# salesforce/warp-drive

Measured on AMD Instinct MI355X. Metric: env steps/sec, TagContinuous 5 taggers x 100 runners, higher is better.
Workload: dtype f32; 1 GPU; BASELINE configs[2]: TagContinuous 5 taggers x 100 runners, partial obs K=10 (F=71), num_envs=2000 per GPU; tick = sample_actions (2 heads) + step + reset of finished replicas (one fused launch); num_envs_per_gpu=2000, num_agents=105, launch_mode=plan, kernels_per_tick=1, ticks_per_launch=1, parallelism=env-replica sharding x1

## Files before the change

### warp_drive_amd/csrc/kernels/tc_fast.h

```cpp
#pragma once
#include "wd_common.h"
#include "tc_fetch.h"
#include "tc_sample.h"
#include "tc_move.h"
#include "tc_tags.h"
#include "tc_reset.h"
#include "tc_knn.h"
#include "tc_rows.h"

namespace {

template <int KMAX, bool FUSED, bool EXACTK, int IDB, bool SAMPLE = FUSED, bool LOOP = false, int SN = 0, int SA = 0,
          int ST = 0>
__device__ __forceinline__ int tc_fast_impl(const TcArgs &a, const TcFuse &fz, unsigned char *smem, int n_acc,
                                            int n_turn, int tick = 0, int n_taggers_in = 0, TcCarry *cy = nullptr,
                                            const TcLoopConsts *lc = nullptr) {
  WD_TC_PROBE_TICK(LOOP, tick);
  const int N = a.N, K = EXACTK ? KMAX : a.K;
  const int F = 7 * K + 1;
  int tid_ = threadIdx.x;
  if constexpr (LOOP) asm volatile("" : "+v"(tid_));
  const int tid = tid_, T_ = WD_TC_BLOCKDIM;
  const int epb = max(1, T_ / N);
  const int n_waves = (T_ + 63) >> 6, wave = __builtin_amdgcn_readfirstlane(tid >> 6), lane = tid & 63;
  const size_t slab_acc_bytes = tc_align16((size_t)4 * epb * N * n_acc);
  const bool compact = (epb == 1);
  const size_t slab_turn_bytes = tc_align16((size_t)4 * epb * N * n_turn);
  const bool one_slab = tc_one_slab(N);
  const TcFastLds l = tc_carve_fast(smem, epb, N, K, n_waves,
                                    !SAMPLE ? 0 : one_slab ? max(slab_acc_bytes, slab_turn_bytes) : slab_acc_bytes + slab_turn_bytes,
                                    compact);
  const TcTables &tb = l.tb;
  float *const slab_acc = (float *)smem, *const slab_turn = (float *)(smem + (one_slab ? 0 : slab_acc_bytes));
  float *const stage = l.stage + (size_t)wave * l.stage_dwords;
  const int el = tid / N, ag = tid - el * N;
  const float invK = 1.0f / (float)K, invN = 1.0f / (float)N;
  const int NP = ((N + 3) & ~3) + 8;

  int group = blockIdx.x;
#ifndef WD_TC_BLOCK_ORDER_PLAIN
  if constexpr (IDB == 7) {
    const int bx = blockIdx.x & 7, bq = gridDim.x >> 3, br = gridDim.x & 7;
    group = bx * bq + min(bx, br) + (int)(blockIdx.x >> 3);
  }
#endif
  const int env0 = a.env_begin + group * epb;
  __builtin_amdgcn_s_setprio(3);
  WD_TC_PROBE_RT(16); WD_TC_PROBE(0); WD_TC_PROBE_HW(21);
  TcIn in;
  bool reloaded = false;
  if constexpr (LOOP) {
    in = cy->in;
    reloaded = cy->reload != 0;
    if (reloaded) {
      tc_load_state(in, a, fz, env0, epb, N, n_acc, n_turn, tid, tick == 0);
      cy->in.type = in.type; cy->in.skill = in.skill; cy->in.step_reward = in.step_reward;
    }
  } else {
    tc_issue_loads<FUSED, SAMPLE>(in, a, fz, env0, epb, N, n_acc, n_turn, tid, slab_acc, slab_turn, true);
  }
  const bool tab_in_lds = (n_acc <= WD_TC_TAB) && (n_turn <= WD_TC_TAB);
  int n_taggers_ = n_taggers_in;
  if constexpr (LOOP) {
    if (tick == 0) n_taggers_ = tc_build_tables(tb, a, N, n_acc, n_turn, tab_in_lds, in);
  } else {
    n_taggers_ = tc_build_tables(tb, a, N, n_acc, n_turn, tab_in_lds, in);
  }
  const int n_taggers = n_taggers_;
  if (env0 >= a.E) return n_taggers;
  if constexpr (!LOOP) WD_TC_PROBE(1);

  const int env = env0 + el;
  const bool active = (el < epb) && (env < a.E);
  const int gi = env * N + ag;
  const int li = tid;
  const int agents_here = min(epb, a.E - env0) * N;
  if constexpr (LOOP) {
    if (active && ag == 0) a.done[env] = 0;
    static_assert(!LOOP || (SN > 0 && SA > 0 && ST == WD_TC_BLOCKDIM), "the multi-tick entry is built for one shape");
    tc_fetch_slabs_straight<SN, SA, ST>(slab_acc, slab_turn, fz.probs_acc, fz.probs_turn, env0, wave, lane);
    WD_TC_PROBE(1);
  }
  int2 sampled = in.sampled;
  const unsigned long long live_mask = __ballot(active && in.sg != 0);
  if constexpr (!LOOP) {
    if (compact && lane == 0) tb.live_cnt[wave] = __popcll(live_mask);
  }
  if constexpr ((IDB != 7) && (KMAX <= 12)) {
    if (compact && tid < 64) tb.cell_cnt[tid] = 0;
  }
  if constexpr (LOOP) {
    static_assert(!LOOP || IDB == 7, "tc_sample_heads_carried samples from two slabs: replicas of at most 128 agents");
    sampled = tc_sample_heads_carried<SA>(fz, in.epoch, cy->k0, cy->k1, active, gi, li, slab_acc, slab_turn, n_acc, n_turn);
    if (compact && lane == 0) tb.live_cnt[wave] = __popcll(live_mask);
  } else if (FUSED) {
    if (active && ag == 0) a.done[env] = 0;
    if (SAMPLE) sampled = tc_sample_heads(a, fz, in, active, gi, li, slab_acc, slab_turn, n_acc, n_turn, env0, epb);
  }
  WD_TC_PROBE(2);
  __syncthreads();
  WD_TC_PROBE(3);
  int my_c = ag, n_live = N;
  if (compact) {
    int before = 0;
    n_live = 0;
    for (int w2 = 0; w2 < n_waves; ++w2) {
      const int c = tb.live_cnt[w2];
      before += (w2 < wave) ? c : 0;
      n_live += c;
    }
    my_c = before + __popcll(live_mask & ((1ull << lane) - 1ull));
  }
  constexpr bool PRE = (IDB != 7) && (KMAX <= 12);
  constexpr bool TIE_TABLE = (IDB != 7);
  bool pre_on = false;
  int cells_C = 0;
  float cell_len = 0.0f, cell_inv = 0.0f;
  int my_cell = 0, my_cell_slot = 0;
  uint4 hint_a = make_uint4(~0u, ~0u, ~0u, ~0u), hint_b = hint_a;
  if constexpr (PRE) {
    pre_on = compact && (a.knn_prev != nullptr) && (n_live >= WD_TC_PRE_MIN_LIVE) && (l.stage_dwords >= WD_TC_LIST_DWORDS);
    if (pre_on && active && in.sg != 0) {
      const uint4 *const h = (const uint4 *)(a.knn_prev + (size_t)(env * N + ag) * 8);
      hint_a = h[0];
      hint_b = h[1];
    }
    if (pre_on) {
      cells_C = tc_cell_grid(n_live, K);
      cell_len = a.grid_length / (float)max(cells_C, 1);
      cell_inv = (float)cells_C / a.grid_length;
    }
  }

  float edge_pen = 0.0f, my_x = 0.0f, my_y = 0.0f;
  const int sg = in.sg;
  const bool is_runner = active && (in.type == 0) && (sg != 0);
  if (active) {
    const TcMoved m = tc_move<LOOP>(a, tb, in, sampled, gi, tab_in_lds, LOOP ? cy : nullptr, LOOP ? lc : nullptr);
    edge_pen = m.edge_pen; my_x = m.x; my_y = m.y;
    if constexpr (LOOP) {
      cy->in.x = m.x; cy->in.y = m.y;
      cy->in.cleared = (sg == 0) ? 1 : 0;
    }
    l.xy[el * NP + ag] = make_float2(sg ? m.x : (PRE && pre_on ? __builtin_nanf("") : WD_BIG), m.y);
    if (compact) {
      if (sg) {
        bool by_cell = false;
        if constexpr (PRE) {
          if (cells_C != 0) {
            const int2 c = tc_cell_xy(m.x, m.y, cell_inv, cells_C);
            my_cell = tc_cell_place(c, cells_C);
            my_cell_slot = atomicAdd(&tb.cell_cnt[my_cell], 1);
            by_cell = true;
          }
        }
        if (!by_cell) {
          l.xyc[my_c] = make_float2(m.x, m.y);
          l.cid[1 + my_c] = (short)ag;
          if (PRE && pre_on) {
            uint4 *const slot = (uint4 *)(l.stage + (size_t)(my_c >> 6) * l.stage_dwords) + 2 * (my_c & 63);
            slot[0] = hint_a;
            slot[1] = hint_b;
          }
        }
      }
      if (ag == 0) {
        l.cid[0] = -1;
        if (PRE && pre_on) {
          l.xyc[n_live] = make_float2(WD_BIG, WD_BIG);
          l.xy[N] = make_float2(__builtin_nanf(""), 0.0f);
        }
      }
    }
    tc_feat_store(l.feat, li, m.ft);
    l.sig[li] = (sg ? 1 : 0) | (in.cleared ? 2 : 0);
    if ((in.cleared != 0) != (sg == 0)) a.obs_rows_cleared[gi] = sg ? 0 : 1;
    l.tagcnt[li] = 0;
    if (ag == 0) {
      const int t = in.tstep + 1;
      a.timestep[env] = t;
      tb.tstep[el] = t;
      if constexpr (LOOP) tb.tfrac[el] = (float)tc_div_const((double)t, (double)a.T, lc->r_T);
      else tb.tfrac[el] = (float)((double)t / (double)a.T);
      if constexpr (LOOP) {
        cy->in.tstep = t;
        if (reloaded) tb.nrun[el] = in.nrun;
      } else {
        tb.nrun[el] = in.nrun;
      }
    }
  }
  WD_TC_PROBE(4);
  __syncthreads();
  WD_TC_PROBE(5);
  int cell_incl = 0;
  if constexpr (PRE) {
    if (cells_C != 0) {
      const int cnt = tb.cell_cnt[lane];
      cell_incl = cnt;
#pragma unroll
      for (int d = 1; d < 64; d <<= 1) {
        const int up = __shfl_up(cell_incl, d, 64);
        cell_incl += (lane >= d) ? up : 0;
      }
      my_c = __builtin_amdgcn_ds_bpermute(my_cell << 2, cell_incl - cnt) + my_cell_slot;
      if (active && sg != 0) {
        l.xyc[my_c] = make_float2(my_x, my_y);
        l.cid[1 + my_c] = (short)ag;
        uint4 *const slot = (uint4 *)(l.stage + (size_t)(my_c >> 6) * l.stage_dwords) + 2 * (my_c & 63);
        slot[0] = hint_a;
        slot[1] = hint_b;
      }
    }
  }

  bool tagged = false;
  if constexpr (LOOP) {
    if (is_runner)
      tagged = tc_find_tag<true>(a, tb, l.xy + el * NP, l.tagcnt + el * N, &tb.nrun[el], n_taggers, my_x, my_y, lc->Bc);
  } else {
    if (is_runner)
      tagged = tc_find_tag(a, tb, l.xy + el * NP, l.tagcnt + el * N, &tb.nrun[el], n_taggers, my_x, my_y);
  }
  if constexpr (PRE) {
    if (cells_C != 0) __syncthreads();
  }

  WD_TC_PROBE(6);
  int nid[KMAX + 1], rank[KMAX + 1];
#pragma unroll
  for (int k = 0; k <= KMAX; ++k) { nid[k] = -1; rank[k] = k; }
  bool in_order = true;
  __builtin_amdgcn_s_setprio(2);
  const bool searcher = compact ? (tid < n_live) : (active && sg != 0);
  const float2 *const sxy = compact ? l.xyc : l.xy + el * NP;
  const int n_cand = compact ? n_live : N;
  int row_agent = ag;
  constexpr int L = KMAX + ((EXACTK && IDB == 7) ? 2 : 3);
  const bool split = compact && (n_waves == 2) && (n_live <= 64) && (n_live >= 16) &&
                     (l.stage_dwords >= 64 * L);
  const int j_half = split ? (((n_live + 7) >> 3) << 2) : n_cand;
  const bool helper = split && (wave == 1);
  unsigned S[L];
  bool prefiltered = false;
  unsigned extra = 0xffffffffu;
  if constexpr (PRE) {
    if (pre_on) {
      unsigned Tb = 0u;
      float sx = 0.0f, sy = 0.0f;
      int2 scell = make_int2(0, 0);
      if (searcher) {
        const uint4 *const slot = (const uint4 *)stage + 2 * lane;
        const uint4 pa = slot[0], pb = slot[1];
        sx = sxy[ag].x; sy = sxy[ag].y;
        Tb = tc_knn_bound16<KMAX>(l.xy, N, sx, sy, pa, pb, K);
        if (cells_C != 0) {
          scell = tc_cell_xy(sx, sy, cell_inv, cells_C);
          Tb = min(Tb, tc_cell_cover2(sx, sy, scell, cell_len, cells_C));
        }
      }
      WD_TC_PROBE(7);
      if (__ballot(searcher) != 0ull && __ballot(searcher && Tb == 0x7f800000u) == 0ull) {
        const float Tf = searcher ? __uint_as_float(Tb) : -1.0f;
#pragma unroll
        for (int k = 0; k < L; ++k) S[k] = 0xffffffffu;
        const int C = cells_C;
        int r = 0, r_end = -1, run0 = 0, run1 = n_cand, x_lo = 0, y_lo = 0, x_hi = 0, y_hi = 0;
        if (C != 0) {
          const int last = min(63, __builtin_amdgcn_readfirstlane(n_live) - 1 - 64 * wave);
          x_lo = __builtin_amdgcn_readfirstlane(scell.x); y_lo = __builtin_amdgcn_readfirstlane(scell.y);
          x_hi = __builtin_amdgcn_readlane(scell.x, last); y_hi = __builtin_amdgcn_readlane(scell.y, last);
          r = max(0, y_lo - 1);
          r_end = min(C - 1, y_hi + 1);
          run1 = 0;
        }
        const TcPreList pl = tc_pre_list(stage, lane);
        int j = 0, j_end = 0;
        int listed = 0, words = 0;
        int probe_trips = 0;
        bool finished = false;
        while (!finished) {
          while (words < WD_TC_LIST_CAP) {
            if (j >= j_end) {
              bool flush = false;
              int p0 = 0, p1 = 0;
              while (!flush && r <= r_end) {
                int lo = C, hi = -1;
                for (int yy = max(y_lo, r - 1); yy <= min(y_hi, r + 1); ++yy) {
                  const bool fwd = (yy & 1) == 0;
                  const int from = (yy == y_lo) ? x_lo : (fwd ? 0 : C - 1), to = (yy == y_hi) ? x_hi : (fwd ? C - 1 : 0);
                  lo = min(lo, min(from, to));
                  hi = max(hi, max(from, to));
                }
                lo = max(0, lo - 1);
                hi = min(C - 1, hi + 1);
                const int first_cell = r * C + ((r & 1) ? C - 1 - hi : lo), last_cell = r * C + ((r & 1) ? C - 1 - lo : hi);
                ++r;
                if (hi < lo) continue;
                const int b = first_cell == 0 ? 0 : __builtin_amdgcn_readlane(cell_incl, max(first_cell, 1) - 1);
                const int e = __builtin_amdgcn_readlane(cell_incl, last_cell);
                const int j0 = max(run1, b & ~3), j1 = min(n_cand, (e + 3) & ~3);
                if (j1 <= j0) continue;
                if (run1 > run0 && j0 != run1) { p0 = run0; p1 = run1; flush = true; run0 = j0; run1 = j1; }
                else if (run1 > run0) run1 = j1;
                else { run0 = j0; run1 = j1; }
              }
              if (!flush) {
                if (run1 <= run0) { finished = true; break; }
                p0 = run0; p1 = run1; run0 = run1;
              }
              j = p0;
              j_end = p1;
            }
            const int j_stop = min(j_end, j + 32 * (WD_TC_LIST_CAP - words));
            tc_pre_pass1(sxy, sx, sy, j, j_stop, Tf, pl, listed);
            words += (j_stop - j + 31) >> 5;
            j = j_stop;
          }
          if (words != 0) tc_pre_pass2<L, IDB>(sxy, sx, sy, pl, listed, S, extra, probe_trips);
          listed = 0;
          words = 0;
        }
        WD_TC_PROBE_VAL(18, probe_trips);
        unsigned sK = S[KMAX];
#pragma unroll
        for (int k = 1; k < KMAX; ++k) sK = (k == K) ? S[k] : sK;
        const bool held = (sK >> IDB) + 2u <= (Tb >> IDB);
        prefiltered = __ballot(searcher && !held) == 0ull;
        WD_TC_PROBE_VAL(19, prefiltered ? 1 : 2);
        if (!prefiltered) extra = 0xffffffffu;
      }
      WD_TC_PROBE(8);
    }
  }
  if (!prefiltered && (searcher || (helper && lane < n_live))) {
    const int me = helper ? lane : ag;
    tc_chain_range<L, IDB>(sxy, sxy[me].x, sxy[me].y, helper ? j_half : 0, helper ? n_cand : j_half, S);
  }
  WD_TC_PROBE(9);
  if (split) {
    if (helper && lane < n_live) {
#pragma unroll
      for (int k = 0; k < L; ++k) ((unsigned *)stage)[64 * k + lane] = S[k];
      __builtin_amdgcn_s_setprio(0);
    }
    __syncthreads();
    if (searcher) {
      const unsigned *const theirs = (const unsigned *)(l.stage + (size_t)l.stage_dwords);
      unsigned P[L];
#pragma unroll
      for (int k = 0; k < L; ++k) P[k] = theirs[64 * k + lane];
      tc_merge_sorted<L>(S, P);
    }
  }
  bool exact = true;
  unsigned zone_hi = 0u;
  if (searcher) {
    unsigned o[L - 1];
    __builtin_amdgcn_s_setprio(1);
    exact = tc_resolve_keys<KMAX, IDB, L, TIE_TABLE>(sxy, ag, K, S, o, nid, rank, in_order, l.cid);
    WD_TC_PROBE(10);
    {
      unsigned oKth = o[KMAX - 1];
#pragma unroll
      for (int k = 0; k < KMAX - 1; ++k) oKth = (k == K - 1) ? o[k] : oKth;
      zone_hi = (oKth >> IDB) + 1u;
    }
    if constexpr (PRE) {
      if (pre_on) {
        unsigned w[8];
#pragma unroll
        for (int q = 0; q < 8; ++q) {
          unsigned pair = 0u;
#pragma unroll
          for (int h = 0; h < 2; ++h) {
            const int k = 2 * q + h;
            const unsigned key = (k < L - 1) ? o[k < L - 1 ? k : 0] : (k == L - 1) ? extra : 0xffffffffu;
            const unsigned id = (key >= 0x7f800000u) ? 0xffffu : (unsigned)(unsigned short)l.cid[1 + (key & ((1u << IDB) - 1u))];
            pair |= id << (16 * h);
          }
          w[q] = pair;
        }
        uint4 *const h = (uint4 *)(a.knn_prev + (size_t)(env * N + l.cid[1 + ag]) * 8);
        h[0] = make_uint4(w[0], w[1], w[2], w[3]);
        h[1] = make_uint4(w[4], w[5], w[6], w[7]);
      }
    }
    if (!exact && !(EXACTK && IDB == 7) && (IDB == 7 || n_cand <= 128)) {
      WD_TC_PROBE_VAL(20, 1);
      int nid2[KMAX], rank2[KMAX];
#pragma unroll
      for (int k = 0; k < KMAX; ++k) { nid2[k] = -1; rank2[k] = k; }
      tc_knn_registers<KMAX>(sxy, ag, n_cand, K, nid2, rank2);
#pragma unroll
      for (int k = 0; k < KMAX; ++k) { nid[k] = nid2[k]; rank[k] = rank2[k]; }
      nid[KMAX] = -1;
      rank[KMAX] = KMAX;
      in_order = false;
      exact = true;
    }
  }
  if constexpr (IDB != 7 || EXACTK) {
    unsigned long long need = __ballot(searcher && !exact);
    if (need != 0ull) {
      WD_TC_PROBE_VAL(20, 1);
      unsigned long long unresolved = 0ull;
      const float mx = searcher ? sxy[ag].x : 0.0f, my = searcher ? sxy[ag].y : 0.0f;
      while (need != 0ull) {
        const int fl = __ffsll((long long)need) - 1;
        need &= need - 1ull;
        const float sx = __builtin_bit_cast(float, __builtin_amdgcn_readlane(__builtin_bit_cast(int, mx), fl));
        const float sy = __builtin_bit_cast(float, __builtin_amdgcn_readlane(__builtin_bit_cast(int, my), fl));
        const unsigned zh = (unsigned)__builtin_amdgcn_readlane((int)zone_hi, fl);
        const int self = __builtin_amdgcn_readlane(ag, fl);
        const float2 *const zxy = compact ? sxy : l.xy + __builtin_amdgcn_readlane(el, fl) * NP;
        const int cnt = tc_zone_resolve<TIE_TABLE>(zxy, n_cand, sx, sy, self, zh, IDB, K, (unsigned char *)stage, lane, l.cid);
        if (cnt > 64) {
          unresolved |= 1ull << fl;
        } else {
          const unsigned short *const out = (const unsigned short *)((const unsigned char *)stage + 128 + 512);
#pragma unroll
          for (int k = 0; k < KMAX; ++k) {
            const int v = (k < K) ? (int)out[k] : -1;
            if (lane == fl) { nid[k] = v; rank[k] = k; }
          }
          if (lane == fl) { nid[KMAX] = -1; rank[KMAX] = KMAX; in_order = false; }
        }
        asm volatile("" ::: "memory");
        __builtin_amdgcn_wave_barrier();
      }
      if ((unresolved >> lane) & 1ull) {
        int nid2[KMAX];
#pragma unroll
        for (int k = 0; k < KMAX; ++k) nid2[k] = -1;
        tc_knn_scan<KMAX, TIE_TABLE>(sxy, ag, n_cand, K, nid2, l.cid);
#pragma unroll
        for (int k = 0; k < KMAX; ++k) { nid[k] = nid2[k]; rank[k] = k; }
        nid[KMAX] = -1;
        rank[KMAX] = KMAX;
        in_order = false;
      }
    }
  }
  if (searcher && compact) {
    row_agent = l.cid[1 + ag];
#pragma unroll
    for (int k = 0; k <= KMAX; ++k) nid[k] = l.cid[1 + nid[k]];
  }
  __builtin_amdgcn_s_setprio(0);
  WD_TC_PROBE(11);

  if constexpr (LOOP) {
    static_assert(!LOOP || (EXACTK && KMAX == 10 && IDB == 7), "the id rows of the multi-tick entry are built for K = 10");
    const bool any_out_of_order = __ballot(!in_order) != 0ull;
    if (searcher) {
      unsigned *const idrow = (unsigned *)(l.ids + row_agent * KMAX);
#pragma unroll
      for (int k = 0; k < KMAX; k += 2) idrow[k >> 1] = ((unsigned)nid[k] & 0xffffu) | ((unsigned)nid[k + 1] << 16);
      if (any_out_of_order && !in_order) {
        unsigned short *const hrow = l.ids + row_agent * KMAX;
#pragma unroll
        for (int k = 0; k <= KMAX; ++k)
          if (rank[k] < KMAX) hrow[rank[k]] = (unsigned short)(nid[k] < 0 ? 0xffff : nid[k]);
#pragma unroll
        for (int k = 0; k < KMAX; ++k) nid[k] = (int)((const short *)hrow)[k];
      }
      tc_store_id_row<false>(a.nearest_ids + (long)env0 * (SN * KMAX), __umul24((unsigned)row_agent, 4u * KMAX), nid);
    }
    if (active && sg == 0 && (reloaded || in.cleared == 0)) {
      int none[KMAX];
#pragma unroll
      for (int k = 0; k < KMAX; ++k) none[k] = -1;
      tc_store_id_row<true>(a.nearest_ids + (long)env0 * (SN * KMAX), __umul24((unsigned)ag, 4u * KMAX), none);
    }
  } else {
    const int ebase = el * N;
    const bool any_out_of_order = __ballot(!in_order) != 0ull;
    if (active && sg == 0) {
      unsigned short *const own = l.ids + (size_t)li * K;
#pragma unroll
      for (int k = 0; k < KMAX; ++k)
        if (k < K) own[k] = 0xffff;
    }
    if (searcher) {
      unsigned short *const idrow = l.ids + (size_t)(ebase + row_agent) * K;
#pragma unroll
      for (int k = 0; k < KMAX; ++k)
        if (k < K) idrow[k] = (unsigned short)(ebase + nid[k]);
      if (any_out_of_order && !in_order) {
#pragma unroll
        for (int k = 0; k <= KMAX; ++k)
          if (rank[k] < K) idrow[rank[k]] = (unsigned short)(nid[k] < 0 ? 0xffff : ebase + nid[k]);
      }
    }
  }
  __syncthreads();
  const int rpw = (agents_here + n_waves - 1) / n_waves;
  const int wrow0 = wave * rpw;
  const int wrows = max(0, min(rpw, agents_here - wrow0));
  if constexpr (!LOOP)
    tc_flush_ids(l.ids + (size_t)wrow0 * K, a.nearest_ids + ((long)env0 * N + wrow0) * K, wrows * K, lane, wrow0, N,
                 invK, invN, epb == 1);
  WD_TC_PROBE(12);
  const int n_live_rows = __popcll(__ballot(lane < wrows && (l.sig[wrow0 + lane] & 1)));
  constexpr int SPARSE_NUM = LOOP ? WD_TC_LOOP_SPARSE_NUM : 9, SPARSE_DEN = 16;
  if (n_live_rows * SPARSE_DEN <= wrows * SPARSE_NUM) {
    if constexpr (LOOP) {
      static_assert(!LOOP || (EXACTK && KMAX == 10), "the descriptor flush of the multi-tick entry is built for K = 10");
      tc_gather_rows_sparse<true, KMAX>(a, l, tb, stage, env0, wrow0, wrows, lane, K, N, invK, invN);
    } else {
      tc_gather_rows_sparse(a, l, tb, stage, env0, wrow0, wrows, lane, K, N, invK, invN);
    }
  } else {
    int R = tc_stage_rows(F, n_waves);
    if constexpr (IDB != 7) {
      R = max(R, min(min(64, (l.stage_dwords - 20) / F), 192 / K));
    }
    constexpr int U = 3;
    int rr[U], so[U];
#pragma unroll
    for (int u = 0; u < U; ++u) {
      const int t = lane + 64 * u;
      rr[u] = (int)(((float)t + 0.5f) * invK);
      so[u] = rr[u] * F + (t - rr[u] * K);
    }
    float *const obs_w = a.obs + ((long)env0 * N + wrow0) * F;
    for (int r0 = 0; r0 < wrows; r0 += R) {
      const int rc = min(R, wrows - r0);
      float *const dst = obs_w + (long)r0 * F;
      const int mis = (int)(((size_t)dst >> 2) & 3);
      const int items = rc * K;
      const unsigned short *const idp = l.ids + (size_t)(wrow0 + r0) * K;
      const int fp = wrow0 + r0;
      int tt[U];
      unsigned jq[U];
#pragma unroll
      for (int u = 0; u < U; ++u) { tt[u] = min(lane + 64 * u, items - 1); jq[u] = idp[tt[u]]; }
      const bool clamped2 = lane + 128 >= items, clamped1 = lane + 64 >= items, clamped0 = lane >= items;
      TcFeat me[U], nb[U];
      int off[U];
#pragma unroll
      for (int u = 0; u < U; ++u) {
        const bool cl = (u == 0) ? clamped0 : (u == 1) ? clamped1 : clamped2;
        const int r_last = rc - 1, o_last = r_last * F + (K - 1);
        const int r = cl ? r_last : rr[u];
        off[u] = cl ? o_last : so[u];
        me[u] = tc_feat_load(l.feat, fp + r);
        const bool valid = ((me[u].type_sig & 1) != 0) && (jq[u] != 0xffffu);
        nb[u] = tc_feat_load(l.feat, valid ? (int)jq[u] : fp + r);
      }
#pragma unroll
      for (int u = 0; u < U; ++u) {
        const bool valid = ((me[u].type_sig & 1) != 0) && (jq[u] != 0xffffu);
        unsigned mv = valid ? 0xffffffffu : 0u;
        asm volatile("" : "+v"(mv));
        const unsigned ts = (unsigned)nb[u].type_sig & mv;
        float *o = stage + mis + off[u];
        o[0] = (float)(nb[u].nx - me[u].nx);
        o[K] = (float)(nb[u].ny - me[u].ny);
        o[2 * K] = nb[u].nsp - me[u].nsp;
        o[3 * K] = nb[u].nac - me[u].nac;
        o[4 * K] = nb[u].ndir - me[u].ndir;
        o[5 * K] = __uint_as_float(ts & 0x3f800000u);
        o[6 * K] = __uint_as_float((0u - (ts & 1u)) & 0x3f800000u);
      }
      if (lane < rc) {
        const int m = wrow0 + r0 + lane;
        const int e_m = (int)(((float)m + 0.5f) * invN);
        stage[mis + lane * F + 7 * K] = (l.sig[m] & 1) ? tb.tfrac[e_m] : 0.0f;
      }
      asm volatile("" ::: "memory");
      __builtin_amdgcn_wave_barrier();
      tc_flush_run(stage, dst, rc * F, lane);
      asm volatile("" ::: "memory");
      __builtin_amdgcn_wave_barrier();
    }
  }
  WD_TC_PROBE(13);
  __syncthreads();
  WD_TC_PROBE(14);

  if (active) tc_finish_agent(a, tb, el, ag, gi, env, sg, is_runner, tagged, l.tagcnt[li], edge_pen, in.step_reward, FUSED);
  if (FUSED) {
    __syncthreads();
    bool any = false;
    for (int e = 0; e < min(epb, a.E - env0); ++e) any = any || (tb.doneflag[e] != 0);
    if constexpr (LOOP) {
      if (active) {
        cy->in.sg = (tagged && a.runner_exits) ? 0 : sg;
        cy->in.epoch = in.epoch + 1u;
      }
      cy->reload = __builtin_amdgcn_readfirstlane(any ? 1 : 0);
    }
    if (any) {
      asm volatile("s_waitcnt vmcnt(0)" ::: "memory");
      __syncthreads();
      tc_reset_finished(a, fz, tb, env0, epb);
      if constexpr (LOOP) {
        asm volatile("s_waitcnt vmcnt(0)" ::: "memory");
        __syncthreads();
      }
    }
  }
  WD_TC_PROBE(15); WD_TC_PROBE_RT(17);
  return n_taggers;
}

template <int KMAX, bool EXACTK, int IDB, int SN, int SA, int ST>
__device__ __forceinline__ void tc_fast_rollout(const TcArgs &a, const TcFuse &fz, unsigned char *smem, int n_acc,
                                                int n_turn, int ticks) {
  int n_taggers = 0;
  TcCarry cy;
  cy.in = TcIn{};
  cy.reload = 1;
  cy.k0 = __builtin_amdgcn_readfirstlane(fz.rng_state[0]);
  cy.k1 = __builtin_amdgcn_readfirstlane(fz.rng_state[1]);
  const TcLoopConsts lc = tc_loop_consts(a.max_speed, a.grid_length, a.T, a.margin);
  for (int tick = 0; tick < ticks; ++tick) {
    n_taggers = tc_fast_impl<KMAX, true, EXACTK, IDB, true, true, SN, SA, ST>(a, fz, smem, n_acc, n_turn, tick, n_taggers, &cy,
                                                                              &lc);
    asm volatile("s_waitcnt vmcnt(0)" ::: "memory");
    __syncthreads();
  }
}

}
```

### warp_drive_amd/csrc/kernels/tc_rows.h

```cpp
#pragma once
#include "wd_common.h"
#include "tc_move.h"

namespace {

__device__ __forceinline__ void tc_flush_run(const float *stage, float *dst, int n, int lane) {
  const int mis = (int)(((size_t)dst >> 2) & 3);
  const int head = min(n, (4 - mis) & 3);
  const int nvec = (n - head) >> 2;
  const int tail0 = head + 4 * nvec;
  typedef float v4f __attribute__((ext_vector_type(4)));
  const v4f *sv = (const v4f *)(stage + mis + head);
  v4f *dv = (v4f *)(dst + head);
#define WD_TC_STORE_WT(ptr, val) asm volatile("global_store_dwordx4 %0, %1, off sc1" ::"v"(ptr), "v"(val) : "memory")
  for (int base = 0; base < nvec; base += 192) {
    const int nrem = nvec - base;
    const int q = base + lane;
    const v4f v0 = sv[min(q, nvec - 1)], v1 = sv[min(q + 64, nvec - 1)], v2 = sv[min(q + 128, nvec - 1)];
    if (nrem >= 64) WD_TC_STORE_WT(&dv[q], v0);
    else if (lane < nrem) WD_TC_STORE_WT(&dv[q], v0);
    if (nrem >= 128) WD_TC_STORE_WT(&dv[q + 64], v1);
    else if (lane + 64 < nrem) WD_TC_STORE_WT(&dv[q + 64], v1);
    if (nrem >= 192) WD_TC_STORE_WT(&dv[q + 128], v2);
    else if (lane + 128 < nrem) WD_TC_STORE_WT(&dv[q + 128], v2);
  }
#undef WD_TC_STORE_WT
  if (lane < head) dst[lane] = stage[mis + lane];
  if (lane < n - tail0) dst[tail0 + lane] = stage[mis + tail0 + lane];
}

__device__ __forceinline__ void tc_flush_ids(const unsigned short *src, int *dst, int n, int lane, int row0, int N,
                                             float invK, float invN, bool one_replica) {
  const int mis = (int)(((size_t)dst >> 2) & 3);
  const int head = min(n, (4 - mis) & 3);
  const int nvec = (n - head) >> 2;
  const int tail0 = head + 4 * nvec;
  auto local = [&](int v, int i) -> int {
    if (one_replica) return v;
    const int row = row0 + (int)(((float)i + 0.5f) * invK);
    const int sub = (int)(((float)row + 0.5f) * invN) * N;
    return v - (v >= 0 ? sub : 0);
  };
  typedef int v4i __attribute__((ext_vector_type(4)));
  for (int q = lane; q < nvec; q += 64) {
    const int i = head + 4 * q;
    const int r0 = (int)(short)src[i], r1 = (int)(short)src[i + 1], r2 = (int)(short)src[i + 2],
              r3 = (int)(short)src[i + 3];
    const v4i v = {local(r0, i), local(r1, i + 1), local(r2, i + 2), local(r3, i + 3)};
    asm volatile("global_store_dwordx4 %0, %1, off sc1" ::"v"(dst + i), "v"(v) : "memory");
  }
  if (lane < head) dst[lane] = local((int)(short)src[lane], lane);
  if (lane < n - tail0) dst[tail0 + lane] = local((int)(short)src[tail0 + lane], tail0 + lane);
}

template <bool DWORD_TAIL, int NN>
__device__ __forceinline__ void tc_store_id_row(int *replica_rows, unsigned row_bytes, const int (&v)[NN]) {
  static_assert(NN >= 10, "a row of ten ids");
  typedef int v4i __attribute__((ext_vector_type(4)));
  typedef int v2i __attribute__((ext_vector_type(2)));
  typedef v4i __attribute__((aligned(8))) v4i_a8;
  typedef v2i __attribute__((aligned(8))) v2i_a8;
  int *const dst = (int *)((char *)replica_rows + row_bytes);
  const v4i q0 = {v[0], v[1], v[2], v[3]}, q1 = {v[4], v[5], v[6], v[7]};
  *(v4i_a8 *)dst = q0;
  *(v4i_a8 *)(dst + 4) = q1;
  if constexpr (DWORD_TAIL) {
    asm volatile("global_store_dword %0, %1, off offset:32" ::"v"(dst), "v"(v[8]) : "memory");
    asm volatile("global_store_dword %0, %1, off offset:36" ::"v"(dst), "v"(v[9]) : "memory");
  } else {
    const v2i q2 = {v[8], v[9]};
    *(v2i_a8 *)(dst + 8) = q2;
  }
}

#define WD_TC_STAGE_TARGET 5400
#ifndef WD_TC_LOOP_SPARSE_NUM
#define WD_TC_LOOP_SPARSE_NUM 9
#endif
__device__ __forceinline__ int tc_stage_rows(int row_dwords, int n_waves) {
  const int target = (n_waves > 4) ? WD_TC_STAGE_TARGET / 2 : WD_TC_STAGE_TARGET;
  return max(1, min(64, target / (4 * row_dwords)));
}

struct TcFastLds {
  TcFeatArrays feat;
  float2 *xy;
  int *sig;
  int *tagcnt;
  float2 *xyc;
  short *cid;
  unsigned short *ids;
  float *stage;
  int stage_dwords;
  TcTables tb;
};

__device__ __forceinline__ TcFastLds tc_carve_fast(unsigned char *p0, int epb, int N, int K, int n_waves,
                                                   size_t min_area_bytes, bool compact) {
  TcFastLds l;
  const size_t A = (size_t)epb * N;
  const int F = 7 * K + 1;
  size_t off = 0;
  l.feat.a = (TcFeatA *)(p0 + off); off += sizeof(TcFeatA) * A;
  l.feat.b = (TcFeatB *)(p0 + off); off += sizeof(TcFeatB) * A;
  l.xy = (float2 *)(p0 + off); off += 8 * (size_t)epb * (((N + 3) & ~3) + 8);
  l.sig = (int *)(p0 + off); off += 4 * A;
  l.tagcnt = (int *)(p0 + off); off += 4 * A;
  l.xyc = l.xy;
  l.cid = nullptr;
  if (compact) {
    off = tc_align16(off);
    l.xyc = (float2 *)(p0 + off); off += 8 * (size_t)(((N + 3) & ~3) + 8);
    l.cid = (short *)(p0 + off); off += tc_align16(2 * ((size_t)N + 1));
  }
  l.ids = (unsigned short *)(p0 + off); off = tc_align16(off + 2 * A * K);
  l.stage_dwords = (int)(tc_align16((size_t)4 * tc_stage_rows(F, n_waves) * F) / 4) + 4 + 16;
  if (compact && N > 128) l.stage_dwords = max(l.stage_dwords, 1152);
  l.stage = (float *)(p0 + off); off += (size_t)4 * l.stage_dwords * n_waves;
  off = tc_align16(off > min_area_bytes ? off : min_area_bytes);
  l.tb = tc_carve_tables(p0 + off, epb, N);
  return l;
}

__device__ __forceinline__ void tc_store_own_dwords(float *rowp, int F, int d0, const float (&v)[4], bool on) {
#pragma unroll
  for (int e = 0; e < 4; ++e)
    if (on && d0 + e >= 0 && d0 + e < F) rowp[d0 + e] = v[e];
}

template <int KC>
struct TcLeanRows {
  static constexpr int F = 7 * KC + 1, SL = (F + 6) & ~3, NV = SL >> 2, RPR = 64 / NV;
  static constexpr int STAGE_DWORDS = (((4 * (WD_TC_STAGE_TARGET / (4 * F)) * F) + 15) & ~15) / 4 + 4 + 16;
  static constexpr int CAP = STAGE_DWORDS - 16;
  static constexpr int RS = (CAP / SL < 192 / KC) ? (CAP / SL < 64 ? CAP / SL : 64) : (192 / KC < 64 ? 192 / KC : 64);
  static constexpr int ACT_NONE = 0, ACT_OWN = 1, ACT_FULL = 2, ACT_MERGE = 3;
  static_assert((RS + 1) * SL + 4 <= STAGE_DWORDS, "the unclamped LDS reads of the flush stay inside the staging buffer");
  static_assert(((RS - 1) / (3 * RPR)) * 3 * RPR + 3 * RPR - 1 <= RS, "highest slot a trip of three rounds reads");
  static_assert(4 * (NV - 2) < F && 4 * (NV - 2) + 4 > F && 4 * (NV - 1) - 1 == F, "tail positions of the descriptor");
  static_assert(4 * (52 * F + 3) < 65536 && NV >= 4 && RPR * NV <= 64, "descriptor fields");
};

__device__ __forceinline__ void tc_store_own_dwords_at(float *p, int F, int d0, const float (&v)[4], bool on) {
#pragma unroll
  for (int e = 0; e < 4; ++e)
    if (on && d0 + e >= 0 && d0 + e < F) p[e] = v[e];
}

template <bool LOOP = false, int KC = 0>
__device__ __forceinline__ void tc_gather_rows_sparse(const TcArgs &a, const TcFastLds &l, const TcTables &tb, float *stage,
                                               int env0, int wrow0, int wrows, int lane, int K_, int N, float invK,
                                               float invN) {
  typedef float v4f __attribute__((ext_vector_type(4)));
  const int K = LOOP ? KC : K_;
  const int F = 7 * K + 1;
  const int SL = (F + 6) & ~3;
  const int NV = SL >> 2;
  const int cap = l.stage_dwords - 16;
  int rs = min(min(64, cap / SL), 192 / K);
  if constexpr (LOOP) rs = TcLeanRows<KC>::RS;
  const int RPR = 64 / NV;
  const float invNV = 1.0f / (float)NV;
  constexpr int U = 3;
  int rr[U], kk[U];
#pragma unroll
  for (int u = 0; u < U; ++u) {
    const int t = lane + 64 * u;
    rr[u] = (int)(((float)t + 0.5f) * invK);
    kk[u] = t - rr[u] * K;
  }
  const int fsub = (int)(((float)lane + 0.5f) * invNV), fv = lane - fsub * NV;
  const int sgv = (lane < wrows) ? l.sig[wrow0 + lane] : 2;
  const unsigned long long lmask = __ballot((sgv & 1) != 0);
  unsigned long long zmask = __ballot(sgv == 0);
  unsigned char *const rowlist = (unsigned char *)(stage + cap);
  if (sgv & 1) rowlist[__popcll(lmask & ((1ull << lane) - 1ull))] = (unsigned char)lane;
  float *const obs_w = a.obs + ((long)env0 * N + wrow0) * F;
  const unsigned bdw = (unsigned)((size_t)obs_w >> 2);
  const unsigned short *const idw = l.ids + (size_t)wrow0 * K;
  const int n_rows = __popcll(lmask);
  while (zmask) {
    const int r = __ffsll((long long)zmask) - 1;
    zmask &= zmask - 1ull;
    float *const rowp = obs_w + (long)r * F;
    const int mis = (int)((bdw + (unsigned)(r * F)) & 3u);
    const int d0 = 4 * lane - mis;
    const float z[4] = {0.0f, 0.0f, 0.0f, 0.0f};
    if (lane < NV) {
      if (d0 >= 0 && d0 + 4 <= F) {
        const v4f q = {0.0f, 0.0f, 0.0f, 0.0f};
        asm volatile("global_store_dwordx4 %0, %1, off sc1" ::"v"(rowp + d0), "v"(q) : "memory");
      } else {
        tc_store_own_dwords(rowp, F, d0, z, true);
      }
    }
  }
  for (int j0 = 0; j0 < n_rows; j0 += rs) {
    const int rc = min(rs, n_rows - j0);
    const int items = rc * K;
    if (lane < rc) {
      const v4f zero = {0.0f, 0.0f, 0.0f, 0.0f};
      v4f *const sl = (v4f *)(stage + lane * SL);
      sl[0] = zero;
      sl[NV - 2] = zero;
      sl[NV - 1] = zero;
    }
#pragma unroll
    for (int u = 0; u < U; ++u) {
      if (64 * u < items) {
        if (lane + 64 * u < items) {
          const int r = rowlist[j0 + rr[u]];
          const unsigned jq = idw[r * K + kk[u]];
          const TcFeat me = tc_feat_load(l.feat, wrow0 + r);
          const bool valid = (jq != 0xffffu);
          const TcFeat nb = tc_feat_load(l.feat, valid ? (int)jq : wrow0 + r);
          unsigned mv = valid ? 0xffffffffu : 0u;
          asm volatile("" : "+v"(mv));
          const unsigned ts = (unsigned)nb.type_sig & mv;
          const int mis = (int)((bdw + (unsigned)(r * F)) & 3u);
          float *o = stage + rr[u] * SL + mis + kk[u];
          o[0] = (float)(nb.nx - me.nx);
          o[K] = (float)(nb.ny - me.ny);
          o[2 * K] = nb.nsp - me.nsp;
          o[3 * K] = nb.nac - me.nac;
          o[4 * K] = nb.ndir - me.ndir;
          o[5 * K] = __uint_as_float(ts & 0x3f800000u);
          o[6 * K] = __uint_as_float((0u - (ts & 1u)) & 0x3f800000u);
        }
      }
    }
    [[maybe_unused]] unsigned desc = 0u;
    if (lane < rc) {
      const int r = rowlist[j0 + lane];
      const int e_m = (int)(((float)(wrow0 + r) + 0.5f) * invN);
      const int mis = (int)((bdw + (unsigned)(r * F)) & 3u);
      stage[lane * SL + mis + 7 * K] = tb.tfrac[e_m];
      if constexpr (LOOP) {
        typedef TcLeanRows<KC> D;
        const bool prev_known = (r > 0), next_known = (r + 1 < wrows);
        const bool prev_live = (((lmask << 1) >> r) & 1ull) != 0ull, next_live = (((lmask >> 1) >> r) & 1ull) != 0ull;
        const unsigned head = (mis == 0)                   ? D::ACT_FULL
                              : (prev_live && lane > 0)    ? D::ACT_NONE
                              : (prev_live || !prev_known) ? D::ACT_OWN
                                                           : D::ACT_FULL;
        const unsigned tail = (next_live && lane + 1 < rc) ? D::ACT_MERGE
                              : (next_live || !next_known) ? D::ACT_OWN
                                                           : D::ACT_FULL;
        const unsigned a_nv2 = (mis == 0) ? tail : (unsigned)D::ACT_FULL, a_nv1 = (mis >= 2) ? tail : (unsigned)D::ACT_NONE;
        desc = head | (a_nv2 << 2) | (a_nv1 << 4) | ((unsigned)D::ACT_FULL << 6) | ((unsigned)mis << 8) |
               ((unsigned)(4 * (r * F - mis + 3)) << 16);
      }
    }
    asm volatile("" ::: "memory");
    __builtin_amdgcn_wave_barrier();
    if constexpr (LOOP) {
      typedef TcLeanRows<KC> D;
      static_assert(D::RPR == 3 && D::NV == 19 && D::F == 71 && D::SL == 76 && D::RS == 17, "built for K = 10");
      constexpr int W = 3;
      const bool idle = (fsub >= D::RPR);
      const int fs = idle ? 0 : fsub;
      const unsigned sh = idle ? 10u : (fv == 0) ? 0u : (fv == D::NV - 2) ? 2u : (fv == D::NV - 1) ? 4u : 6u;
      for (int sb = 0; sb < rc; sb += W * D::RPR) {
        unsigned dd[W];
        v4f q[W], nx[W];
#pragma unroll
        for (int u = 0; u < W; ++u)
          dd[u] = (unsigned)__builtin_amdgcn_ds_bpermute(4 * (sb + u * D::RPR + fs), (int)desc);
#pragma unroll
        for (int u = 0; u < W; ++u) {
          q[u] = *(const v4f *)(stage + (sb + u * D::RPR + fs) * D::SL + 4 * fv);
          nx[u] = *(const v4f *)(stage + (sb + u * D::RPR + fs + 1) * D::SL);
        }
#pragma unroll
        for (int u = 0; u < W; ++u) {
          if (sb + u * D::RPR < rc) {
            const unsigned act = (dd[u] >> sh) & 3u;
            const unsigned voff = (dd[u] >> 16) + 16u * (unsigned)fv;
            unsigned mm = (act == (unsigned)D::ACT_MERGE) ? 0xffffffffu : 0u;
            asm volatile("" : "+v"(mm));
            v4f o = q[u];
            o.x = __uint_as_float(__float_as_uint(o.x) | (__float_as_uint(nx[u].x) & mm));
            o.y = __uint_as_float(__float_as_uint(o.y) | (__float_as_uint(nx[u].y) & mm));
            o.z = __uint_as_float(__float_as_uint(o.z) | (__float_as_uint(nx[u].z) & mm));
            o.w = __uint_as_float(__float_as_uint(o.w) | (__float_as_uint(nx[u].w) & mm));
            if (act >= (unsigned)D::ACT_FULL)
              asm volatile("global_store_dwordx4 %0, %1, %2 offset:-12 sc1" ::"v"(voff), "v"(o), "s"(obs_w) : "memory");
            if (__ballot(act == (unsigned)D::ACT_OWN) != 0ull) {
              const float vals[4] = {o.x, o.y, o.z, o.w};
              const int d0 = 4 * fv - (int)((dd[u] >> 8) & 3u);
              tc_store_own_dwords_at((float *)((char *)obs_w + voff) - 3, F, d0, vals, act == (unsigned)D::ACT_OWN);
            }
          }
        }
      }
      asm volatile("" ::: "memory");
      __builtin_amdgcn_wave_barrier();
      continue;
    }
    for (int sb = 0; sb < rc; sb += 3 * RPR) {
      constexpr int W = 3;
      int slot[W], r[W], d0[W];
      bool on[W];
#pragma unroll
      for (int u = 0; u < W; ++u) {
        slot[u] = sb + u * RPR + fsub;
        on[u] = (fsub < RPR) && (slot[u] < rc);
        slot[u] = min(slot[u], rc - 1);
        r[u] = rowlist[j0 + slot[u]];
      }
      v4f q[W], nx[W];
#pragma unroll
      for (int u = 0; u < W; ++u) {
        const int mis = (int)((bdw + (unsigned)(r[u] * F)) & 3u);
        d0[u] = 4 * fv - mis;
        q[u] = *(const v4f *)(stage + slot[u] * SL + 4 * fv);
        nx[u] = *(const v4f *)(stage + min(slot[u] + 1, rc - 1) * SL);
      }
#pragma unroll
      for (int u = 0; u < W; ++u) {
        if (sb + u * RPR < rc) {
          float *const rowp = obs_w + (long)r[u] * F;
          const bool head_part = on[u] && (d0[u] < 0), tail_part = on[u] && (d0[u] < F) && (d0[u] + 4 > F);
          const bool prev_known = (r[u] > 0), next_known = (r[u] + 1 < wrows);
          const bool prev_live = prev_known && ((lmask >> (r[u] - 1)) & 1ull);
          const bool next_live = next_known && ((lmask >> (r[u] + 1)) & 1ull);
          const bool merge_next = tail_part && next_live && (slot[u] + 1 < rc);
          unsigned mm = merge_next ? 0xffffffffu : 0u;
          asm volatile("" : "+v"(mm));
          v4f o = q[u];
          o.x = __uint_as_float(__float_as_uint(o.x) | (__float_as_uint(nx[u].x) & mm));
          o.y = __uint_as_float(__float_as_uint(o.y) | (__float_as_uint(nx[u].y) & mm));
          o.z = __uint_as_float(__float_as_uint(o.z) | (__float_as_uint(nx[u].z) & mm));
          o.w = __uint_as_float(__float_as_uint(o.w) | (__float_as_uint(nx[u].w) & mm));
          const bool skip = head_part && prev_live && (slot[u] > 0);
          const bool own_only = (head_part && !skip && (prev_live || !prev_known)) ||
                                (tail_part && !merge_next && (next_live || !next_known));
          const bool full = on[u] && (d0[u] < F) && !skip && !own_only;
          if (full) asm volatile("global_store_dwordx4 %0, %1, off sc1" ::"v"(rowp + d0[u]), "v"(o) : "memory");
          if (__ballot(own_only) != 0ull) {
            const float vals[4] = {o.x, o.y, o.z, o.w};
            tc_store_own_dwords(rowp, F, d0[u], vals, own_only);
          }
        }
      }
    }
    asm volatile("" ::: "memory");
    __builtin_amdgcn_wave_barrier();
  }
}

}
```

Baseline: 124.4 million env_steps/s.

## Add lean dense observation-row gather for the multi-tick loop path

Result: faster. 127.5 million env_steps/s, median of 6 (+2.5%).

```diff
diff --git a/warp_drive_amd/csrc/kernels/tc_fast.h b/warp_drive_amd/csrc/kernels/tc_fast.h
--- a/warp_drive_amd/csrc/kernels/tc_fast.h
+++ b/warp_drive_amd/csrc/kernels/tc_fast.h
@@ -502,7 +502,8 @@
     tc_flush_ids(l.ids + (size_t)wrow0 * K, a.nearest_ids + ((long)env0 * N + wrow0) * K, wrows * K, lane, wrow0, N,
                  invK, invN, epb == 1);
   WD_TC_PROBE(12);
-  const int n_live_rows = __popcll(__ballot(lane < wrows && (l.sig[wrow0 + lane] & 1)));
+  const unsigned long long live_rows = __ballot(lane < wrows && (l.sig[wrow0 + lane] & 1));
+  const int n_live_rows = __popcll(live_rows);
   constexpr int SPARSE_NUM = LOOP ? WD_TC_LOOP_SPARSE_NUM : 9, SPARSE_DEN = 16;
   if (n_live_rows * SPARSE_DEN <= wrows * SPARSE_NUM) {
     if constexpr (LOOP) {
@@ -511,6 +512,9 @@
     } else {
       tc_gather_rows_sparse(a, l, tb, stage, env0, wrow0, wrows, lane, K, N, invK, invN);
     }
+  } else if constexpr (LOOP) {
+    static_assert(!LOOP || (EXACTK && KMAX == 10 && IDB == 7 && SN > 64 && SN <= 128), "two wavefronts, one replica per block");
+    tc_gather_rows_dense_lean<KMAX, SN>(a, l, tb, stage, env0, wave, lane, live_rows);
   } else {
     int R = tc_stage_rows(F, n_waves);
     if constexpr (IDB != 7) {
diff --git a/warp_drive_amd/csrc/kernels/tc_rows.h b/warp_drive_amd/csrc/kernels/tc_rows.h
--- a/warp_drive_amd/csrc/kernels/tc_rows.h
+++ b/warp_drive_amd/csrc/kernels/tc_rows.h
@@ -4,8 +4,7 @@
 
 namespace {
 
-__device__ __forceinline__ void tc_flush_run(const float *stage, float *dst, int n, int lane) {
-  const int mis = (int)(((size_t)dst >> 2) & 3);
+__device__ __forceinline__ void tc_flush_run_at(const float *stage, float *dst, int mis, int n, int lane) {
   const int head = min(n, (4 - mis) & 3);
   const int nvec = (n - head) >> 2;
   const int tail0 = head + 4 * nvec;
@@ -27,6 +26,9 @@
 #undef WD_TC_STORE_WT
   if (lane < head) dst[lane] = stage[mis + lane];
   if (lane < n - tail0) dst[tail0 + lane] = stage[mis + tail0 + lane];
+}
+__device__ __forceinline__ void tc_flush_run(const float *stage, float *dst, int n, int lane) {
+  tc_flush_run_at(stage, dst, (int)(((size_t)dst >> 2) & 3), n, lane);
 }
 
 __device__ __forceinline__ void tc_flush_ids(const unsigned short *src, int *dst, int n, int lane, int row0, int N,
@@ -195,6 +197,14 @@
       }
     }
   }
+  [[maybe_unused]] int fs = 0;
+  [[maybe_unused]] unsigned sh = 0u;
+  if constexpr (LOOP) {
+    typedef TcLeanRows<KC> D;
+    const bool idle = (fsub >= D::RPR);
+    fs = idle ? 0 : fsub;
+    sh = idle ? 10u : (fv == 0) ? 0u : (fv == D::NV - 2) ? 2u : (fv == D::NV - 1) ? 4u : 6u;
+  }
   for (int j0 = 0; j0 < n_rows; j0 += rs) {
     const int rc = min(rs, n_rows - j0);
     const int items = rc * K;
@@ -205,38 +215,15 @@
       sl[NV - 2] = zero;
       sl[NV - 1] = zero;
     }
-#pragma unroll
-    for (int u = 0; u < U; ++u) {
-      if (64 * u < items) {
-        if (lane + 64 * u < items) {
-          const int r = rowlist[j0 + rr[u]];
-          const unsigned jq = idw[r * K + kk[u]];
-          const TcFeat me = tc_feat_load(l.feat, wrow0 + r);
-          const bool valid = (jq != 0xffffu);
-          const TcFeat nb = tc_feat_load(l.feat, valid ? (int)jq : wrow0 + r);
-          unsigned mv = valid ? 0xffffffffu : 0u;
-          asm volatile("" : "+v"(mv));
-          const unsigned ts = (unsigned)nb.type_sig & mv;
-          const int mis = (int)((bdw + (unsigned)(r * F)) & 3u);
-          float *o = stage + rr[u] * SL + mis + kk[u];
-          o[0] = (float)(nb.nx - me.nx);
-          o[K] = (float)(nb.ny - me.ny);
-          o[2 * K] = nb.nsp - me.nsp;
-          o[3 * K] = nb.nac - me.nac;
-          o[4 * K] = nb.ndir - me.ndir;
-          o[5 * K] = __uint_as_float(ts & 0x3f800000u);
-          o[6 * K] = __uint_as_float((0u - (ts & 1u)) & 0x3f800000u);
-        }
-      }
-    }
     [[maybe_unused]] unsigned desc = 0u;
-    if (lane < rc) {
-      const int r = rowlist[j0 + lane];
-      const int e_m = (int)(((float)(wrow0 + r) + 0.5f) * invN);
-      const int mis = (int)((bdw + (unsigned)(r * F)) & 3u);
-      stage[lane * SL + mis + 7 * K] = tb.tfrac[e_m];
-      if constexpr (LOOP) {
-        typedef TcLeanRows<KC> D;
+    if constexpr (LOOP) {
+      typedef TcLeanRows<KC> D;
+      unsigned rw = 0u;
+      if (lane < rc) {
+        const int r = rowlist[j0 + lane];
+        const int mis = (int)((bdw + (unsigned)(r * F)) & 3u);
+        stage[lane * SL + mis + 7 * K] = tb.tfrac[0];
+        rw = (unsigned)r | ((unsigned)mis << 10);
         const bool prev_known = (r > 0), next_known = (r + 1 < wrows);
         const bool prev_live = (((lmask << 1) >> r) & 1ull) != 0ull, next_live = (((lmask >> 1) >> r) & 1ull) != 0ull;
         const unsigned head = (mis == 0)                   ? D::ACT_FULL
@@ -250,6 +237,61 @@
         desc = head | (a_nv2 << 2) | (a_nv1 << 4) | ((unsigned)D::ACT_FULL << 6) | ((unsigned)mis << 8) |
                ((unsigned)(4 * (r * F - mis + 3)) << 16);
       }
+#pragma unroll
+      for (int u = 0; u < U; ++u) {
+        if (64 * u < items) {
+          const unsigned w = (unsigned)__builtin_amdgcn_ds_bpermute(4 * rr[u], (int)rw);
+          if (lane + 64 * u < items) {
+            const int r = (int)(w & 0xffu);
+            const unsigned jq = idw[r * K + kk[u]];
+            const TcFeat me = tc_feat_load(l.feat, wrow0 + r);
+            const bool valid = (jq != 0xffffu);
+            const TcFeat nb = tc_feat_load(l.feat, valid ? (int)jq : wrow0 + r);
+            unsigned mv = valid ? 0xffffffffu : 0u;
+            asm volatile("" : "+v"(mv));
+            const unsigned ts = (unsigned)nb.type_sig & mv;
+            float *o = (float *)((char *)(stage + rr[u] * SL + kk[u]) + (w >> 8));
+            o[0] = (float)(nb.nx - me.nx);
+            o[K] = (float)(nb.ny - me.ny);
+            o[2 * K] = nb.nsp - me.nsp;
+            o[3 * K] = nb.nac - me.nac;
+            o[4 * K] = nb.ndir - me.ndir;
+            o[5 * K] = __uint_as_float(ts & 0x3f800000u);
+            o[6 * K] = __uint_as_float((0u - (ts & 1u)) & 0x3f800000u);
+          }
+        }
+      }
+    } else {
+#pragma unroll
+      for (int u = 0; u < U; ++u) {
+        if (64 * u < items) {
+          if (lane + 64 * u < items) {
+            const int r = rowlist[j0 + rr[u]];
+            const unsigned jq = idw[r * K + kk[u]];
+            const TcFeat me = tc_feat_load(l.feat, wrow0 + r);
+            const bool valid = (jq != 0xffffu);
+            const TcFeat nb = tc_feat_load(l.feat, valid ? (int)jq : wrow0 + r);
+            unsigned mv = valid ? 0xffffffffu : 0u;
+            asm volatile("" : "+v"(mv));
+            const unsigned ts = (unsigned)nb.type_sig & mv;
+            const int mis = (int)((bdw + (unsigned)(r * F)) & 3u);
+            float *o = stage + rr[u] * SL + mis + kk[u];
+            o[0] = (float)(nb.nx - me.nx);
+            o[K] = (float)(nb.ny - me.ny);
+            o[2 * K] = nb.nsp - me.nsp;
+            o[3 * K] = nb.nac - me.nac;
+            o[4 * K] = nb.ndir - me.ndir;
+            o[5 * K] = __uint_as_float(ts & 0x3f800000u);
+            o[6 * K] = __uint_as_float((0u - (ts & 1u)) & 0x3f800000u);
+          }
+        }
+      }
+      if (lane < rc) {
+        const int r = rowlist[j0 + lane];
+        const int e_m = (int)(((float)(wrow0 + r) + 0.5f) * invN);
+        const int mis = (int)((bdw + (unsigned)(r * F)) & 3u);
+        stage[lane * SL + mis + 7 * K] = tb.tfrac[e_m];
+      }
     }
     asm volatile("" ::: "memory");
     __builtin_amdgcn_wave_barrier();
@@ -257,9 +299,6 @@
       typedef TcLeanRows<KC> D;
       static_assert(D::RPR == 3 && D::NV == 19 && D::F == 71 && D::SL == 76 && D::RS == 17, "built for K = 10");
       constexpr int W = 3;
-      const bool idle = (fsub >= D::RPR);
-      const int fs = idle ? 0 : fsub;
-      const unsigned sh = idle ? 10u : (fv == 0) ? 0u : (fv == D::NV - 2) ? 2u : (fv == D::NV - 1) ? 4u : 6u;
       for (int sb = 0; sb < rc; sb += W * D::RPR) {
         unsigned dd[W];
         v4f q[W], nx[W];
@@ -349,4 +388,79 @@
   }
 }
 
-}
+template <int KC, int SN>
+struct TcLeanDense {
+  static constexpr int F = 7 * KC + 1;
+  static constexpr int R = WD_TC_STAGE_TARGET / (4 * F);
+  static constexpr int ROWS0 = (SN + 1) / 2, ROWS1 = SN - ROWS0;
+  static constexpr int NCH = (ROWS0 + R - 1) / R;
+  static constexpr int LAST0 = ROWS0 - (NCH - 1) * R, LAST1 = ROWS1 - (NCH - 1) * R;
+  static_assert(R >= 1 && R <= 32 && R * KC <= 192 && R * KC > 128, "at most three items per lane; bit tests on 32 bits");
+  static_assert((ROWS1 + R - 1) / R == NCH && LAST1 >= 1 && LAST1 <= LAST0 && LAST0 <= R, "both wavefronts: NCH chunks");
+  static_assert(LAST1 * KC > 128, "the first two items of a lane exist in every chunk");
+  static_assert(4 * R * F + 12 <= WD_TC_STAGE_TARGET + 16, "a chunk image at any alignment fits the staging buffer");
+};
+
+template <int KC, int SN>
+__device__ __forceinline__ void tc_gather_rows_dense_lean(const TcArgs &a, const TcFastLds &l, const TcTables &tb,
+                                                          float *stage, int env0, int wave, int lane,
+                                                          unsigned long long live) {
+  typedef TcLeanDense<KC, SN> D;
+  constexpr int K = KC, F = D::F, R = D::R, U = 3;
+  const int wrow0 = wave * D::ROWS0;
+  const int last_rows = wave ? D::LAST1 : D::LAST0;
+  int t0[U], r0[U], s0[U];
+#pragma unroll
+  for (int u = 0; u < U; ++u) {
+    t0[u] = lane + 64 * u;
+    r0[u] = (int)((unsigned)t0[u] / (unsigned)K);
+    s0[u] = r0[u] * F + (t0[u] - r0[u] * K);
+  }
+  float *dst = a.obs + ((long)env0 * SN + wrow0) * F;
+  int mis = (int)(((size_t)dst >> 2) & 3);
+  const unsigned short *idp = l.ids + wrow0 * K;
+  int fp = wrow0;
+  const float tfrac = tb.tfrac[0];
+#pragma nounroll
+  for (int c = 0; c < D::NCH; ++c) {
+    const int rc = (c == D::NCH - 1) ? last_rows : R;
+    const bool past = lane + 128 >= rc * K;
+    const int tt[U] = {t0[0], t0[1], past ? t0[1] : t0[2]}, rr[U] = {r0[0], r0[1], past ? r0[1] : r0[2]},
+              so[U] = {s0[0], s0[1], past ? s0[1] : s0[2]};
+    const unsigned lv = (unsigned)live;
+    unsigned jq[U];
+#pragma unroll
+    for (int u = 0; u < U; ++u) jq[u] = idp[tt[u]];
+#pragma unroll
+    for (int u = 0; u < U; ++u) {
+      const int m = fp + rr[u];
+      const TcFeat me = tc_feat_load(l.feat, m);
+      const bool valid = (((lv >> rr[u]) & 1u) != 0u) && (jq[u] != 0xffffu);
+      const TcFeat nb = tc_feat_load(l.feat, valid ? (int)jq[u] : m);
+      unsigned mv = valid ? 0xffffffffu : 0u;
+      asm volatile("" : "+v"(mv));
+      const unsigned ts = (unsigned)nb.type_sig & mv;
+      float *o = stage + mis + so[u];
+      o[0] = (float)(nb.nx - me.nx);
+      o[K] = (float)(nb.ny - me.ny);
+      o[2 * K] = nb.nsp - me.nsp;
+      o[3 * K] = nb.nac - me.nac;
+      o[4 * K] = nb.ndir - me.ndir;
+      o[5 * K] = __uint_as_float(ts & 0x3f800000u);
+      o[6 * K] = __uint_as_float((0u - (ts & 1u)) & 0x3f800000u);
+    }
+    if (lane < rc) stage[mis + lane * F + 7 * K] = ((lv >> lane) & 1u) ? tfrac : 0.0f;
+    asm volatile("" ::: "memory");
+    __builtin_amdgcn_wave_barrier();
+    tc_flush_run_at(stage, dst, mis, rc * F, lane);
+    asm volatile("" ::: "memory");
+    __builtin_amdgcn_wave_barrier();
+    dst += R * F;
+    mis = (mis + R * F) & 3;
+    idp += R * K;
+    fp += R;
+    live >>= R;
+  }
+}
+
+}
```
